# guokiddo1/speech_enhancement

Hardware: AMD Instinct MI355X
Metric: NoiseSup frames/sec (16 kHz, hop 80, 256-pt rfft, two-stage Wiener), batched (higher is better)
Workload: dtype f32; 1 GPU; BASELINE configs[1]: 1024-utterance batch per GPU, 256-pt rfft + two-stage Wiener NoiseSup (etsi_denoise semantics), SURVEY 8(d) synthetic 16 kHz corpus, 2-6 s utterances; utterances_per_gpu=1024, devices_visible=1

## Files before the change

### speech_enhancement_amd/csrc/ns6_beat_plan.h

```cpp
#ifndef SEA_NS6_BEAT_PLAN_H
#define SEA_NS6_BEAT_PLAN_H

#if defined(__HIPCC__) || defined(__CUDACC__)
#define SEA_NS6_HD __host__ __device__
#else
#define SEA_NS6_HD
#endif

namespace sea {
namespace ns6plan {

constexpr int kNoOnset = 0x7fffffff;
constexpr int kDepth = 9;

enum Role { FA = 0, FB = 1, B0 = 2, N1 = 3, G1 = 4, S = 5, kRoles = 6 };

constexpr unsigned kAlways = 0u, kFd = 1u, kLight = 2u, kDifg1 = 4u;
constexpr unsigned kRedeal = 8u;
constexpr unsigned kVariantPlain = kLight | kDifg1, kVariantDense = 0u, kVariantFd = kFd | kLight | kDifg1;
constexpr unsigned kVariantDenseRedeal = kRedeal;
constexpr unsigned kBin64 = 16u;
constexpr unsigned kVariantDenseBin64 = kRedeal | kBin64;
constexpr unsigned kIdctS = 32u;
constexpr unsigned kVariantDenseIdct = kRedeal | kBin64 | kIdctS;
constexpr int kDepthIdct = 12;

struct Flag {
    int d;
    int k;
    unsigned when;
};
constexpr int kMaxFlags = 5;
struct RolePlan {
    int n;
    Flag f[kMaxFlags];
    int ahead;
    int settle;
};

constexpr RolePlan kPlan[kRoles] = {
    {4, {{0, 3, kAlways}, {3, 5, kAlways}, {2, 1, kLight}, {3, 3, kRedeal}, {0, 0, 0}}, 1, 0},
    {2, {{1, 3, kAlways}, {4, 5, kAlways}, {0, 0, 0}, {0, 0, 0}, {0, 0, 0}}, 0, 0},
    {2, {{2, 3, kAlways}, {6, 5, kBin64}, {0, 0, 0}, {0, 0, 0}, {0, 0, 0}}, 0, 0},
    {3, {{5, 5, kAlways}, {7, 5, kAlways}, {2, 1, kRedeal}, {0, 0, 0}, {0, 0, 0}}, 0, 0},
    {1, {{8, 5, kAlways}, {0, 0, 0}, {0, 0, 0}, {0, 0, 0}, {0, 0, 0}}, 0, 0},
    {5, {{1, 1, kAlways}, {3, 3, kAlways}, {6, 5, kAlways}, {kDepth, 5, kAlways}, {kDepth, 5, kFd}}, 0, 1},
};

constexpr RolePlan kPlanIdct[kRoles] = {
    {3, {{0, 3, kAlways}, {4, 5, kAlways}, {4, 3, kAlways}, {0, 0, 0}, {0, 0, 0}}, 1, 0},
    {2, {{1, 3, kAlways}, {5, 5, kAlways}, {0, 0, 0}, {0, 0, 0}, {0, 0, 0}}, 0, 0},
    {2, {{2, 3, kAlways}, {7, 5, kAlways}, {0, 0, 0}, {0, 0, 0}, {0, 0, 0}}, 0, 0},
    {3, {{2, 1, kAlways}, {6, 5, kAlways}, {8, 5, kAlways}, {0, 0, 0}, {0, 0, 0}}, 0, 0},
    {2, {{9, 5, kAlways}, {11, 5, kAlways}, {0, 0, 0}, {0, 0, 0}, {0, 0, 0}}, 0, 0},
    {5, {{1, 1, kAlways}, {3, 3, kAlways}, {7, 5, kAlways}, {10, 5, kAlways}, {kDepthIdct, 5, kAlways}}, 0, 1},
};
SEA_NS6_HD constexpr const RolePlan &plan_of(unsigned variant, int role) { return (variant & kIdctS) ? kPlanIdct[role] : kPlan[role]; }
SEA_NS6_HD constexpr int depth_of(unsigned variant) { return (variant & kIdctS) ? kDepthIdct : kDepth; }

SEA_NS6_HD constexpr bool flag_applies(const Flag &f, unsigned variant) { return f.when == kAlways || (f.when & variant) != 0u; }

SEA_NS6_HD constexpr bool has_flag(unsigned variant, int role, int d, int k)
{
    const RolePlan &p = plan_of(variant, role);
    for (int j = 0; j < p.n; ++j)
        if (p.f[j].d == d && p.f[j].k == k && flag_applies(p.f[j], variant)) return true;
    return false;
}

SEA_NS6_HD constexpr int steady_lead(unsigned variant, int role)
{
    const RolePlan &p = plan_of(variant, role);
    int lead = 0;
    for (int j = 0; j < p.n; ++j) {
        const Flag &f = p.f[j];
        if (flag_applies(f, variant) && f.d + f.k - 1 > lead) lead = f.d + f.k - 1;
    }
    return lead + p.settle;
}
SEA_NS6_HD constexpr int steady_tail(unsigned variant, int role)
{
    const RolePlan &p = plan_of(variant, role);
    int tail = depth_of(variant);
    for (int j = 0; j < p.n; ++j) {
        const Flag &f = p.f[j];
        if (flag_applies(f, variant) && f.d < tail) tail = f.d;
    }
    return tail - p.ahead;
}

SEA_NS6_HD constexpr int steady_begin(unsigned variant, int role, int onset)
{
    return onset == kNoOnset ? kNoOnset : onset + steady_lead(variant, role);
}
SEA_NS6_HD constexpr int steady_end(unsigned variant, int role, int nfr)
{
    const int e = nfr + steady_tail(variant, role);
    return e > 0 ? e : 0;
}

}
}

#undef SEA_NS6_HD
#endif
```

### speech_enhancement_amd/csrc/ns_core.h

```cpp
#pragma once
#include "sea_device.h"
#include "sea_kernels.h"

namespace sea {

namespace {

constexpr int kRing = 320;
constexpr double kLn2 = 0.69314718055994530942;

struct __attribute__((aligned(16))) BackLds {
    float wbuf[68];
    float sbuf[68];
    float sq[80];
    float mel[28];
    float fir[20];
};

struct __attribute__((aligned(16))) NsLds {
    float ring[2][kRing];
    float work[256];
    float psd[68];
    BackLds back;
    float outb[80];
// ... 1359 lines not shown
    B.wbuf[lane] = WLo;
    if (lane == 0) B.wbuf[64] = WHi;
    wave_sync();
    float melOut = ns_mel_fb(B, C, lane);
    melOut = (float)((double)(alfaGF * melOut) + (1.0 - (double)alfaGF) * 1.0);
    float d0, d1;
    lastIn = ns_fir_dif_rl(fir_taps_rl(ns_idct_tap_rl_batch(melOut, C.irWin, lane, idctLds)), buf, lane, lastIn, d0, d1);
    if (lane < 40) *reinterpret_cast<float2 *>(dif + 2 * lane) = make_float2(d0, d1);
    wave_sync();
}

constexpr int kIdctRecFloats = 40;
__device__ __forceinline__ void ns_fir_from_idct_rec(const float *rec, float irWin, const float *buf, int lane, float &y0, float &y1)
{
    const int l = (lane <= 8) ? lane : 8;
    ns_fir_regs(fir_taps_rl(rec[28 + l] * irWin), buf, lane, y0, y1);
}
__device__ __forceinline__ void ns_fir_from_idct_taps(const float *taps, const float *buf, int lane, float &y0, float &y1)
{
    const FirTaps T = fir_taps_rl(taps[kIdsTapStride * lane]);
    constexpr int kFirst = 5;
    float x[18];
    int o = 72 + 2 * ((lane < 40) ? lane : 39);
#pragma unroll
    for (int m = 8; m < 18; m += 2) {
        const float2 v = *reinterpret_cast<const float2 *>(buf + o + m);
        x[m] = v.x;
        x[m + 1] = v.y;
    }
    __builtin_amdgcn_sched_barrier(0);
    y0 = 0.0f, y1 = 0.0f;
#pragma unroll
    for (int k = 0; k < kFirst; ++k) {
        const float c = T.t[8 - k];
        y0 += c * x[16 - k];
        y1 += c * x[17 - k];
    }
    asm("" : "+v"(o) : "v"(y0));
#pragma unroll
    for (int m = 0; m < 8; m += 2) {
        const float2 v = *reinterpret_cast<const float2 *>(buf + o + m);
        x[m] = v.x;
        x[m + 1] = v.y;
    }
    __builtin_amdgcn_sched_barrier(0);
#pragma unroll
    for (int k = kFirst; k < SEA_NTAP; ++k) {
        const float c = T.t[k < 8 ? 8 - k : k - 8];
        y0 += c * x[16 - k];
        y1 += c * x[17 - k];
    }
}

template <int ST, bool FD = false>
__device__ __forceinline__ void ns_stage(NsLds &L, NsRegs &s, const NsConst &C, int lane, NsFd *fd = nullptr,
                                         int *fdFlags = nullptr)
{
    ns_front(L.ring[ST], L.work, L.psd, C.fft, C.win, lane);
    ns_back<ST, false, FD, false, -1, true>(L.psd, L.ring[ST], L.back, s, C, (ST == 0) ? (L.ring[1] + 240) : L.outb, lane, 0.0f, nullptr,
                           nullptr, fd, fdFlags);
}

__device__ __forceinline__ bool dc_filter(const float *dif, float *out, float &yState, int lane)
{
    const float y0 = yState;
    float y = y0;
#pragma unroll 5
    for (int n = 0; n < SEA_HOP; n += 4) {
        const float4 d = *reinterpret_cast<const float4 *>(&dif[n]);
        float4 o;
        y = __fmaf_rn(0.9990234375f, y, d.x);
        o.x = y;
        y = __fmaf_rn(0.9990234375f, y, d.y);
        o.y = y;
        y = __fmaf_rn(0.9990234375f, y, d.z);
        o.z = y;
        y = __fmaf_rn(0.9990234375f, y, d.w);
        o.w = y;
        *reinterpret_cast<float4 *>(&out[n]) = o;
    }
    wave_sync();
    bool unsafe = false;
#pragma unroll
    for (int k = 0; k < 2; ++k) {
        const int n = lane + 64 * k;
        if (n < SEA_HOP) {
            const float ad = fabsf(dif[n]);
            const float ay = fabsf(n == 0 ? y0 : out[n - 1]);
            const bool ok = (ad == 0.0f) || (ay == 0.0f) ||
                            (ay >= ad * 0x1p-16f && ay <= ad * 0x1p26f && ad < 0x1p100f && ad > 0x1p-100f);
            unsafe |= !ok;
        }
    }
    const bool redo = __ballot(unsafe) != 0ull;
    if (redo) {
        wave_sync();
        y = y0;
        for (int n = 0; n < SEA_HOP; ++n) {
            y = (float)__fma_rn(0.9990234375, (double)y, (double)dif[n]);
            out[n] = y;
        }
    }
    yState = y;
    wave_sync();
    return redo;
}
// ... 295 lines not shown
```

### speech_enhancement_amd/csrc/ns_pipe6_kernel.hip

```cpp
#include "ns_core.h"
#include "ns6_beat_plan.h"

namespace sea {

namespace p6 {

#ifdef SEA_NS6_TIMING
__device__ unsigned long long g_ns6_timing[16];
struct RoleTimer6 {
    unsigned long long work = 0, wait = 0, t0 = 0, t1 = 0;
    __device__ __forceinline__ void begin() { t0 = clock64(); }
    __device__ __forceinline__ void mid() { t1 = clock64(); work += t1 - t0; }
    __device__ __forceinline__ void end() { wait += clock64() - t1; }
};
#define NS6_T_DECL RoleTimer6 rt_
#define NS6_T_BEGIN rt_.begin()
#define NS6_T_MID rt_.mid()
#define NS6_T_END rt_.end()
#define NS6_T_FLUSH(r, n) do { if (blockIdx.x == 0 && (threadIdx.x & 63) == 0) { g_ns6_timing[2 * (r)] = rt_.work; g_ns6_timing[2 * (r) + 1] = rt_.wait; g_ns6_timing[12] = (unsigned long long)(n); } } while (0)
#else
#define NS6_T_DECL
#define NS6_T_BEGIN
#define NS6_T_MID
#define NS6_T_END
#define NS6_T_FLUSH(r, n)
#endif

constexpr int kSlots = 8;
constexpr int kSlots1 = 16;
constexpr int kSlotLen = SEA_HOP;
constexpr int kCirc = kSlots * kSlotLen;
constexpr int kCirc1 = kSlots1 * kSlotLen;
constexpr int kMirror = 3 * kSlotLen;
constexpr int kWaves = 6;
constexpr int kDepth = ns6plan::kDepth;
constexpr int kSChunks = 10;
constexpr int kPrioStep = 16;
constexpr int kPrioLevels = 32;
constexpr int kDefaultPerm = 0014352;
constexpr int kRedealPerm = 0140325;

constexpr int kNoOnset = ns6plan::kNoOnset;
constexpr long long kMaxFrames = 0x7fffffffLL - 16;
__device__ __forceinline__ void onset_poll(int &onset, const int *word)
{
    if (onset == kNoOnset)
        onset = __builtin_amdgcn_readfirstlane(__hip_atomic_load(word, __ATOMIC_RELAXED, __HIP_MEMORY_SCOPE_WORKGROUP));
}
__device__ __forceinline__ int tick_of(int f, int onset) { return (int)((unsigned)f - (unsigned)onset + 1u); }
__device__ __forceinline__ bool tick_ge(int f, int k, int onset, int nfr) { return f < nfr && f - (k - 1) >= onset; }

template <bool B>
struct BoolC {
    static constexpr bool value = B;
};
template <unsigned VARIANT, int ROLE, int D, int K, bool STEADY>
__device__ __forceinline__ bool beat_flag(int i, int onset, int nfr)
{
    static_assert(ns6plan::has_flag(VARIANT, ROLE, D, K), "a flag the beat plan of ns6_beat_plan.h does not know");
    return STEADY || tick_ge(i - D, K, onset, nfr);
}
struct NoEnter {
    __device__ __forceinline__ int operator()(int h) const { return h; }
};
template <bool STEADY_LOOP, unsigned VARIANT, int ROLE, bool PAIRED = false, class Beat, class Enter = NoEnter>
__device__ __forceinline__ void run_beats(int niter, int nfr, const int &onset, Beat &&beat, Enter &&enter = Enter{})
{
    int i = 0;
    while (i < niter) {
        if (STEADY_LOOP && i >= ns6plan::steady_begin(VARIANT, ROLE, onset)) {
            const int e0 = ns6plan::steady_end(VARIANT, ROLE, nfr), e = e0 < niter ? e0 : niter;
            if constexpr (PAIRED) {
                if ((i & 1) == 0) {
                    int h = enter(i >> 1);
                    for (const int he = e >> 1; h < he; ++h) {
                        beat(BoolC<true>{}, 2 * h);
                        beat(BoolC<true>{}, 2 * h + 1);
                    }
                    i = 2 * h;
                }
            } else
                for (; i < e; ++i) beat(BoolC<true>{}, i);
        }
        if (i < niter) {
            beat(BoolC<false>{}, i);
            ++i;
        }
    }
}

constexpr int kP1Ring = 8;
constexpr int kRnRing = 4;
constexpr int kW1Ring = 4;
struct __attribute__((aligned(16))) RecPsd {
    float psd[68];
};
struct __attribute__((aligned(16))) RecDen {
    float den[68];
};
struct __attribute__((aligned(16))) RecN {
    float P[68], noise[68];
};
struct __attribute__((aligned(16))) RecOut {
    float out[80];
};

struct __attribute__((aligned(16))) RecTap {
    float rec[kIdctRecFloats];
};

struct __attribute__((aligned(16))) Pipe6Lds {
    float circ0[kCirc + kMirror];
    float circ1[kCirc1 + kMirror];
    float work[2][512];
    BackLds back[2];
    float ssq[80], sdif[80], sout[80], szero[4];
    float frameEn[kSlots], denSum[kSlots];
    int onset;
    float frameEnLog[kSlots];
    int fdFlags[kSlots];
    float idctT[SEA_NMEL * 16];
    RecPsd p0[2], p1[kP1Ring];
    RecDen rd[2];
    RecN rn[kRnRing];
    RecOut ro[2];
    float nzSum[2], alfa[2];
    RecTap tap[2];
    float w1hi[kW1Ring];
};
constexpr bool lds_slots_differ(size_t a, size_t b) { return (a % 256) != (b % 256); }
#define NS6_OFF(m) offsetof(Pipe6Lds, m)
static_assert(lds_slots_differ(NS6_OFF(ssq), NS6_OFF(rd[0].den)) && lds_slots_differ(NS6_OFF(ssq), NS6_OFF(rd[1].den)), "ssq | den");
static_assert(lds_slots_differ(NS6_OFF(sdif), NS6_OFF(rn[0].noise)) && lds_slots_differ(NS6_OFF(sdif), NS6_OFF(rn[1].noise)) &&
              lds_slots_differ(NS6_OFF(sdif), NS6_OFF(rn[2].noise)) && lds_slots_differ(NS6_OFF(sdif), NS6_OFF(rn[3].noise)), "sdif | noise");
static_assert(lds_slots_differ(NS6_OFF(ro[0].out), NS6_OFF(rn[1].noise)) && lds_slots_differ(NS6_OFF(ro[0].out), NS6_OFF(rn[3].noise)) &&
              lds_slots_differ(NS6_OFF(ro[1].out), NS6_OFF(rn[0].noise)) && lds_slots_differ(NS6_OFF(ro[1].out), NS6_OFF(rn[2].noise)), "ro | noise");
static_assert(lds_slots_differ(NS6_OFF(ssq[68]), NS6_OFF(szero)) && lds_slots_differ(NS6_OFF(ssq[72]), NS6_OFF(szero)) &&
              lds_slots_differ(NS6_OFF(ssq[76]), NS6_OFF(szero)), "ssq tail | szero");
static_assert(lds_slots_differ(NS6_OFF(sdif[68]), NS6_OFF(szero)) && lds_slots_differ(NS6_OFF(sdif[72]), NS6_OFF(szero)) &&
              lds_slots_differ(NS6_OFF(sdif[76]), NS6_OFF(szero)), "sdif tail | szero");
static_assert(lds_slots_differ(NS6_OFF(ro[0].out[68]), NS6_OFF(szero)) && lds_slots_differ(NS6_OFF(ro[0].out[72]), NS6_OFF(szero)) &&
              lds_slots_differ(NS6_OFF(ro[0].out[76]), NS6_OFF(szero)) && lds_slots_differ(NS6_OFF(ro[1].out[68]), NS6_OFF(szero)) &&
              lds_slots_differ(NS6_OFF(ro[1].out[72]), NS6_OFF(szero)) && lds_slots_differ(NS6_OFF(ro[1].out[76]), NS6_OFF(szero)), "ro tail | szero");
#undef NS6_OFF
static_assert(sizeof(Pipe6Lds) == 24960 && 4 * sizeof(Pipe6Lds) <= 160 * 1024 && sizeof(Pipe6Lds) < 40 * 1024,
              "the figure in the comment at kP1Ring; four workgroups fit a CU");

struct __attribute__((aligned(16))) Pipe6Idct {
    float tap[2][2][kIdsTapFloats];
    float pad0[4];
    float zeros[kIdsZeros];
    float pad[4];
    float prod[2][2][kIdctProdFloats];
};
constexpr int kIdctBasisAt = 3;
struct __attribute__((aligned(16))) Pipe6LdsIdct {
    Pipe6Lds base;
    Pipe6Idct x;
};
constexpr size_t lds_slot(size_t off) { return (off / 16) % 16; }
constexpr bool lds_group_ok(size_t ssq, size_t den, size_t recA, size_t recB, int r0, int r1)
{
    size_t sl[11] = {lds_slot(ssq), lds_slot(den)};
    int n = 2;
    for (int r = 0; r < 9; ++r) sl[n++] = lds_slot(((r >= r0 && r < r1) ? recA : recB) + r * kIdctStride * sizeof(float));
    for (int i = 0; i < n; ++i)
        for (int j = i + 1; j < n; ++j)
            if (sl[i] == sl[j]) return false;
    return true;
}
#define NS6_OFF(m) offsetof(Pipe6LdsIdct, m)
static_assert(NS6_OFF(base) == 0 && NS6_OFF(x.prod) % 256 == NS6_OFF(x.prod[0][1]) % 256 && NS6_OFF(x.prod) % 256 == NS6_OFF(x.prod[1][0]) % 256 &&
                  NS6_OFF(x.prod) % 256 == NS6_OFF(x.prod[1][1]) % 256 && NS6_OFF(x.prod) % 16 == 0 && (kIdctRow * sizeof(float)) % 16 == 0 &&
                  (NS6_OFF(base.idctT) + kIdctBasisAt * sizeof(float)) % 16 == 0 && kIdctBasisAt + kIdctBasisFloats <= SEA_NMEL * 16 &&
                  NS6_OFF(x.tap[0][1]) % 16 == 0 && NS6_OFF(x.tap[1][1]) + kIdsTapReach * sizeof(float) <= sizeof(Pipe6LdsIdct),
              "the four product records share their slots");
static_assert(lds_group_ok(NS6_OFF(base.ssq), NS6_OFF(base.rd[0].den), NS6_OFF(x.prod[0][0]), NS6_OFF(x.prod[1][1]), 0, 3) &&
                  lds_group_ok(NS6_OFF(base.ssq), NS6_OFF(base.rd[0].den), NS6_OFF(x.prod[0][0]), NS6_OFF(x.prod[1][1]), 3, 9) &&
                  lds_group_ok(NS6_OFF(base.ssq), NS6_OFF(base.rd[1].den), NS6_OFF(x.prod[0][1]), NS6_OFF(x.prod[1][0]), 0, 3) &&
                  lds_group_ok(NS6_OFF(base.ssq), NS6_OFF(base.rd[1].den), NS6_OFF(x.prod[0][1]), NS6_OFF(x.prod[1][0]), 3, 9) &&
                  (kIdctStride * sizeof(float)) % 16 == 0, "n < 28: ssq, den | the rows, in both groups and both parities");
static_assert(NS6_OFF(x.zeros) % 16 == 0 && lds_slots_differ(NS6_OFF(x.zeros) + 256 - kIdctRow * sizeof(float), NS6_OFF(base.ssq)) &&
                  lds_slots_differ(NS6_OFF(x.zeros) + 256 - kIdctRow * sizeof(float), NS6_OFF(base.rd[0].den)) &&
                  lds_slots_differ(NS6_OFF(x.zeros) + 256 - kIdctRow * sizeof(float), NS6_OFF(base.rd[1].den)), "28 <= n: the rows' zeros | ssq, den");
static_assert(lds_slots_differ(NS6_OFF(x.zeros) + 512 - 68 * sizeof(float), NS6_OFF(base.ssq)) &&
                  lds_slots_differ(NS6_OFF(x.zeros) + 512 - 68 * sizeof(float), NS6_OFF(base.sdif)) &&
                  lds_slots_differ(NS6_OFF(x.zeros) + 512 - 68 * sizeof(float), NS6_OFF(x.zeros) + 256 - kIdctRow * sizeof(float)),
              "68 <= n: the den and noise lanes' zeros | ssq, sdif, the rows' zeros");
#undef NS6_OFF
static_assert(4 * sizeof(Pipe6LdsIdct) <= 160 * 1024 && 5 * sizeof(Pipe6LdsIdct) <= 160 * 1024, "four workgroups fit a CU; five, for the compiler's occupancy of 7");

template <int SLOTS>
__device__ __forceinline__ int window_base(int tick) { return ((tick - 3) & (SLOTS - 1)) * kSlotLen; }

template <int SLOTS>
__device__ __forceinline__ void slot_store(float *circ, int tick, int lane, float a, float b)
{
    const int slot = tick & (SLOTS - 1);
    float *p = circ + slot * kSlotLen + 2 * lane;
    *reinterpret_cast<float2 *>(p) = make_float2(a, b);
    if (slot < 3) *reinterpret_cast<float2 *>(p + SLOTS * kSlotLen) = make_float2(a, b);
}

__device__ __forceinline__ void block_sync()
{
    __builtin_amdgcn_fence(__ATOMIC_RELEASE, "workgroup", "local");
    __builtin_amdgcn_s_barrier();
    __builtin_amdgcn_fence(__ATOMIC_ACQUIRE, "workgroup", "local");
}

__device__ __forceinline__ void load_back_const(NsConst &C, const sea_ns_tables *t, int lane)
{
    C.melStart = t->melStart[lane];
    C.melLen = t->melLen[lane];
#pragma unroll
    for (int i = 0; i < SEA_MEL_TAPS; ++i) C.melW[i] = t->melW[i][lane];
    C.irWin = t->irWin[lane];
    C.eps = t->eps;
}

template <bool FD, bool LIGHT , bool DIFG1 ,
          bool STEADY_LOOP ,
          bool REDEAL = false ,
          bool BIN64 = false ,
          bool IDCTS = false ,
          bool PAIRED = false >
__device__ __forceinline__ void ns_pipe6_body(const NsBatchArgs &a, Pipe6Lds &L, Pipe6Idct *X = nullptr)
{
    static_assert(!REDEAL || (!LIGHT && !DIFG1), "the re-deal is a variant of the dense body");
    static_assert(!BIN64 || (REDEAL && !FD), "the guest of B0's second component is a variant of the re-dealt dense body");
    static_assert(!IDCTS || BIN64, "the IDCT sums in the helper wave are a variant of that body in turn");
    static_assert(!PAIRED || STEADY_LOOP, "the paired beats are the steady copies'");
    constexpr unsigned V = (FD ? ns6plan::kFd : 0u) | (LIGHT ? ns6plan::kLight : 0u) | (DIFG1 ? ns6plan::kDifg1 : 0u) | (REDEAL ? ns6plan::kRedeal : 0u) |
                           (BIN64 ? ns6plan::kBin64 : 0u) | (IDCTS ? ns6plan::kIdctS : 0u);
    static_assert(!BIN64 || V == (IDCTS ? ns6plan::kVariantDenseIdct : ns6plan::kVariantDenseBin64),
                  "the variants tests/test_ns6_idct_plan_cpu.py and tests/test_ns6_bin64_plan_cpu.py sweep");
    constexpr int kS1 = IDCTS ? 1 : 0;
    constexpr int DEPTH = ns6plan::depth_of(V);
    static_assert(DEPTH == (IDCTS ? 12 : kDepth), "the depth the ring depths at kP1Ring are derived for");
    constexpr bool LOG_N1 = REDEAL, FIR_FA = REDEAL;
    const int lane = threadIdx.x & 63;
    const int role = ((a.perm6 ? a.perm6 : (REDEAL ? kRedealPerm : kDefaultPerm)) >> (3 * __builtin_amdgcn_readfirstlane(threadIdx.x >> 6))) & 7;
    const int u = a.order ? a.order[blockIdx.x] : (int)blockIdx.x;
    const long long off = a.offsets[u];
    const long long nfr64 = a.lengths[u] / SEA_HOP;
    const int nfr = __builtin_amdgcn_readfirstlane((int)(nfr64 < kMaxFrames ? nfr64 : kMaxFrames));
    const int niter = nfr + DEPTH;
    const bool lrpt = a.prio_row > 0 && a.order;
    const long long longestFr = lrpt ? a.lengths[a.order[0]] / SEA_HOP : 0;
    const float lrptScale = (float)kPrioLevels / (float)(longestFr > 0 ? longestFr : 1);
    const int lrptBias = lrpt ? (int)blockIdx.x / a.prio_row : 0;
    auto prio_by_remaining = [&](int i) {
        if ((FD ? lrpt : true) && (i & (kPrioStep - 1)) == 0) {
            if constexpr (!FD) {
                asm volatile("");
                if (!lrpt) return;
            }
            const int L = __builtin_amdgcn_readfirstlane((int)((float)(nfr - i) * lrptScale)) + lrptBias;
            const int pr = (L + (int)(((unsigned)i / kPrioStep) & (kPrioLevels / 4 - 1))) / (kPrioLevels / 4);
            if (pr >= 3) __builtin_amdgcn_s_setprio(3);
            else if (pr == 2) __builtin_amdgcn_s_setprio(2);
            else if (pr == 1) __builtin_amdgcn_s_setprio(1);
            else __builtin_amdgcn_s_setprio(0);
        }
    };

    {
        static_assert(offsetof(Pipe6Lds, circ0) == 0 && offsetof(Pipe6Lds, circ1) == sizeof(float) * (kCirc + kMirror), "circ0 | circ1 lead the record");
        float *z = reinterpret_cast<float *>(&L);
        for (int i = threadIdx.x; i < kCirc + kCirc1 + 2 * kMirror; i += 64 * kWaves) z[i] = 0.0f;
    }
    if constexpr (!IDCTS)
        for (int i = threadIdx.x; i < SEA_NMEL * 16; i += 64 * kWaves) L.idctT[i] = a.tables->idct[i >> 4][i & 15];
    float *const basisQ = L.idctT + kIdctBasisAt;
    if (threadIdx.x < 4) L.szero[threadIdx.x] = 0.0f;
    if (threadIdx.x < kSlots) {
        L.frameEn[threadIdx.x] = 0.0f;
        L.frameEnLog[threadIdx.x] = 0.0f;
        L.denSum[threadIdx.x] = 0.0f;
    }
    if (threadIdx.x < 2) {
        const int k = threadIdx.x;
        L.rd[k].den[65] = L.rd[k].den[66] = L.rd[k].den[67] = 0.0f;
        L.nzSum[k] = L.alfa[k] = 0.0f;
    }
    if (threadIdx.x < kRnRing) {
        const int k = threadIdx.x;
        L.rn[k].noise[65] = L.rn[k].noise[66] = L.rn[k].noise[67] = 0.0f;
    }
    if (threadIdx.x == 0) L.onset = kNoOnset;
    if constexpr (IDCTS) {
        for (int i = threadIdx.x; i < kIdctBasisFloats; i += 64 * kWaves) {
            const int t = i / kIdctRow, f = i % kIdctRow;
            basisQ[i] = (t < 9 && f < SEA_NMEL) ? a.tables->idct[f][t] : 0.0f;
        }
        if (threadIdx.x < kIdsZeros) X->zeros[threadIdx.x] = 0.0f;
        if (threadIdx.x < 6) L.back[threadIdx.x / 3].mel[SEA_NMEL + threadIdx.x % 3] = 0.0f;
    }
    block_sync();
    NS6_T_DECL;

    if (role == 0) {
        Fft2Regs fft;
        load_fft2_regs<false>(fft, &a.tables->fft, lane, nullptr);
        float win8[8];
#pragma unroll
        for (int k = 0; k < 8; ++k) win8[k] = a.tables->win8[k][lane];
        const float irWin = (FIR_FA && !IDCTS) ? a.tables->irWin[lane] : 0.0f;
        const uint32_t *in32 = reinterpret_cast<const uint32_t *>(a.in + off);
        uint32_t nextw = (lane < 40 && nfr > 0) ? in32[lane] : 0u;
        int onsetG = kNoOnset;
        int onsetS = kNoOnset;
        typedef const __attribute__((address_space(1))) uint32_t *FramePtr;
        unsigned long long nextFr = 0;
        auto beat = [&](auto steady, int i) __attribute__((always_inline)) {
            constexpr bool STEADY = decltype(steady)::value;
            int &onset = *(STEADY && PAIRED ? &onsetS : &onsetG);
            constexpr bool NEXT_S = STEADY && PAIRED;
            NS6_T_BEGIN;
            prio_by_remaining(i);
            if constexpr (LIGHT) {
                if (beat_flag<V, ns6plan::FA, 2, 1, STEADY>(i, onset, nfr)) {
                    const int e = (tick_of(i - 2, onset) + 2) & (kSlots - 1);
                    const float en = vad_frame_energy(L.frameEn[e]);
                    if (lane == 0) L.frameEnLog[e] = en;
                }
            }
            int tick = 0;
            bool actA = false;
            if (STEADY || i < nfr) {
                const uint32_t w = nextw;
                if constexpr (!NEXT_S)
                    if ((STEADY || i + 1 < nfr) && lane < 40) nextw = (in32 + (long long)(i + 1) * 40)[lane];
                if (!STEADY && onset == kNoOnset && __ballot(w != 0u) != 0ull) {
                    onset = i;
                    if (lane == 0) __hip_atomic_store(&L.onset, i, __ATOMIC_RELAXED, __HIP_MEMORY_SCOPE_WORKGROUP);
                }
                if (STEADY || i >= onset) {
                    tick = tick_of(i, onset);
                    const float x0 = (float)(short)(w & 0xFFFFu), x1 = (float)(short)(w >> 16);
                    if (lane < 40) {
                        if constexpr (NEXT_S) nextw = reinterpret_cast<FramePtr>(nextFr)[lane];
                        slot_store<kSlots>(L.circ0, tick, lane, x0, x1);
                    }
                    if constexpr (NEXT_S) {
                        nextFr += SEA_HOP * 2u;
                        asm("" : "+s"(nextFr));
                    }
                    static_assert(ns6plan::has_flag(V, ns6plan::FA, 0, 3), "frame i exists here: its flag is the tick alone");
                    actA = STEADY || tick >= 3;
                }
            }
            const int t1 = tick_of(i - 3 - kS1, onset);
            const bool actB = beat_flag<V, ns6plan::FA, 3 + kS1, 5, STEADY>(i, onset, nfr);
            if constexpr (FIR_FA) {
                if (beat_flag<V, ns6plan::FA, 3 + kS1, 3, STEADY>(i, onset, nfr)) {
                    float y0, y1;
                    if constexpr (IDCTS)
                        ns_fir_from_idct_taps(X->tap[0][(i - 4) & 1], L.circ0 + window_base<kSlots>(t1), lane, y0, y1);
                    else
                        ns_fir_from_idct_rec(L.tap[(i - 3) & 1].rec, irWin, L.circ0 + window_base<kSlots>(t1), lane, y0, y1);
                    if (lane < 40) slot_store<kSlots1>(L.circ1, t1, lane, y0, y1);
                    wave_sync();
                }
            }
            if (actA || actB) {
                wave_sync();
                float e[8];
                ns_window8(L.circ0 + window_base<kSlots>(tick), actA, L.circ1 + window_base<kSlots1>(t1), actB, win8, lane, e);
                if constexpr (STEADY && PAIRED && !FD) {
#pragma unroll
                    for (int q = 0; q < 4; ++q) asm volatile("" : "+v"(fft.head8[q]));
                }
                rfft256_dual_lo<false>(e, L.work[i & 1], fft);
            }
            NS6_T_MID;
            block_sync();
            NS6_T_END;
        };
        run_beats<STEADY_LOOP, V, ns6plan::FA, PAIRED>(niter, nfr, onsetG, beat, [&](int h) {
            onsetS = __builtin_amdgcn_readfirstlane(onsetG);
            const int hs = __builtin_amdgcn_readfirstlane(h);
            unsigned long long fr = reinterpret_cast<unsigned long long>(in32 + (unsigned long long)(unsigned)(2 * hs + 1) * 40u);
            asm("" : "+s"(fr));
            nextFr = fr;
            return hs;
        });
        NS6_T_FLUSH(role, niter);
        if (FD && a.onset_out && lane == 0) a.onset_out[u] = onsetG == kNoOnset ? nfr : onsetG;
    } else if (role == 1) {
        Fft2Regs fft;
        load_fft2_regs<false>(fft, &a.tables->fft, lane, nullptr);
        int onset = kNoOnset;
        auto beat = [&](auto steady, int i) __attribute__((always_inline)) {
            constexpr bool STEADY = decltype(steady)::value;
            NS6_T_BEGIN;
            prio_by_remaining(i);
            if (!STEADY) onset_poll(onset, &L.onset);
            const int g = i - 1;
            if (STEADY || g >= 0) {
                const int f0 = g, f1 = g - 3 - kS1;
                const bool actA = beat_flag<V, ns6plan::FB, 1, 3, STEADY>(i, onset, nfr);
                const bool actB = beat_flag<V, ns6plan::FB, 4 + kS1, 5, STEADY>(i, onset, nfr);
                float *work = L.work[g & 1];
                if (actA || actB) {
                    float o[8];
                    rfft256_dual_hi_keep_last<false>(work, fft, o);
                    psd_from_last_level(o, fft, L.p0[f0 & 1].psd, actA, L.p1[f1 & (kP1Ring - 1)].psd, actB, lane);
// ... 39 lines not shown
                if constexpr (IDCTS) {
                    ns_back<0, true, FD, true, SEA_NMEL, false, true, true, true>(r.psd, nullptr, L.back[0], s, C, X->prod[0][f & 1], lane, frameEn, o.den,
                                                                                  basisQ, &fd, &bits, nullptr, nullptr, nullptr, &x);
                } else if constexpr (BIN64) {
                    ns_back<0, true, FD, true, SEA_NMEL, false, true, true>(r.psd, nullptr, L.back[0], s, C, L.tap[f & 1].rec, lane, frameEn, o.den,
                                                                            L.idctT, &fd, &bits, nullptr, nullptr, nullptr, &x);
                } else if constexpr (FIR_FA) {
                    ns_back<0, true, FD, true, SEA_NMEL, false, true>(r.psd, nullptr, L.back[0], s, C, L.tap[f & 1].rec, lane, frameEn, o.den, L.idctT,
                                                         &fd, &bits);
                    if (FD && lane == 0) L.fdFlags[t & (kSlots - 1)] = bits;
                } else {
                    float y01[2] = {0.0f, 0.0f};
                    ns_back<0, true, FD, true, -1, false, true>(r.psd, L.circ0 + window_base<kSlots>(t), L.back[0], s, C, nullptr, lane, frameEn, o.den,
                                               L.idctT, &fd, &bits, nullptr, y01);
                    if (FD && lane == 0) L.fdFlags[t & (kSlots - 1)] = bits;
                    if (lane < 40) slot_store<kSlots1>(L.circ1, t, lane, y01[0], y01[1]);
                }
            }
            if constexpr (BIN64) {
                if (x.live) {
                    if (!x.done) {
                        const float W = gain_bin<false>(sqrtf(x.P1[64]), sqrtf(x.psd1[64]), x.noise1[64], x.den);
                        x.W = W;
                    }
                    if (lane == 1) L.w1hi[g & (kW1Ring - 1)] = x.W;
                }
            }
            NS6_T_MID;
            block_sync();
            NS6_T_END;
        };
        run_beats<STEADY_LOOP, V, ns6plan::B0, PAIRED>(niter, nfr, onset, beat);
        NS6_T_FLUSH(role, niter);
    } else if (role == 3) {
        const float eps = a.tables->eps;
        NsRegs s;
        regs_init(s, eps);
        int onset = kNoOnset;
        auto beat = [&](auto steady, int i) __attribute__((always_inline)) {
            constexpr bool STEADY = decltype(steady)::value;
            NS6_T_BEGIN;
            prio_by_remaining(i);
            if (!STEADY) onset_poll(onset, &L.onset);
            const int f = i - 5 - kS1, fg = i - 7 - kS1;
            if constexpr (LOG_N1) {
                if (beat_flag<V, ns6plan::N1, 2, 1, STEADY>(i, onset, nfr)) {
                    const int e = (tick_of(i - 2, onset) + 2) & (kSlots - 1);
                    const float en = vad_frame_energy(L.frameEn[e]);
                    if (lane == 0) L.frameEnLog[e] = en;
                }
            }
            if (beat_flag<V, ns6plan::N1, 7 + kS1, 5, STEADY>(i, onset, nfr)) {
                const int t = tick_of(fg, onset);
                s.denEn0 = L.denSum[(t - 2) & (kSlots - 1)];
                s.denEn1 = L.denSum[(t - 1) & (kSlots - 1)];
                s.denEn2 = L.denSum[t & (kSlots - 1)];
                const int nbNow = s.nbFrame[1];
                s.nbFrame[1] = t - 4;
                gain_fact_update(s, L.nzSum[fg & 1]);
                s.nbFrame[1] = nbNow;
                if (lane == 0) L.alfa[fg & 1] = s.alfaGF;
            }
            if (beat_flag<V, ns6plan::N1, 5 + kS1, 5, STEADY>(i, onset, nfr)) {
                const RecPsd &r = L.p1[f & (kP1Ring - 1)];
                RecN &o = L.rn[f & (kRnRing - 1)];
                ns_noise1<BIN64>(r.psd, o.P, o.noise, s, eps, lane);
            }
            NS6_T_MID;
            block_sync();
            NS6_T_END;
        };
        run_beats<STEADY_LOOP, V, ns6plan::N1, PAIRED>(niter, nfr, onset, beat);
        NS6_T_FLUSH(role, niter);
    } else if (role == 4) {
        NsConst C;
        load_back_const(C, a.tables, lane);
        NsRegs s;
        regs_init(s, C.eps);
        float lastIn = 0.0f;
        int onset = kNoOnset;
        auto beat = [&](auto steady, int i) __attribute__((always_inline)) {
            constexpr bool STEADY = decltype(steady)::value;
            NS6_T_BEGIN;
            prio_by_remaining(i);
            if (!STEADY) onset_poll(onset, &L.onset);
            const int f = i - 8 - kS1;
            if constexpr (IDCTS) {
                const int ff = i - 11;
                if (beat_flag<V, ns6plan::G1, 11, 5, STEADY>(i, onset, nfr))
                    ns_fir_from_taps(X->tap[1][ff & 1], L.back[1].fir, L.circ1 + window_base<kSlots1>(tick_of(ff, onset)), L.ro[ff & 1].out, lane);
            }
            if (beat_flag<V, ns6plan::G1, 8 + kS1, 5, STEADY>(i, onset, nfr)) {
                const float *psd = L.p1[f & (kP1Ring - 1)].psd;
                const RecN &r = L.rn[f & (kRnRing - 1)];
                RecOut &o = L.ro[f & 1];
                const int t = tick_of(f, onset);
                const float alfa = L.alfa[f & 1];
                const float *w64 = BIN64 ? &L.w1hi[f & (kW1Ring - 1)] : nullptr;
                if constexpr (IDCTS)
                    ns_gain1_products(psd, r.P, r.noise, alfa, L.back[1], s, C, X->prod[1][f & 1], lane, basisQ, w64);
                else if (DIFG1)
                    ns_gain1_dif(psd, r.P, r.noise, alfa, L.circ1 + window_base<kSlots1>(t), L.back[1], s, C, o.out, lane, L.idctT, lastIn);
                else
                    ns_gain1<BIN64>(psd, r.P, r.noise, alfa, L.circ1 + window_base<kSlots1>(t), L.back[1], s, C, o.out, lane, L.idctT, w64);
            }
            NS6_T_MID;
            block_sync();
            NS6_T_END;
        };
        run_beats<STEADY_LOOP, V, ns6plan::G1, PAIRED>(niter, nfr, onset, beat);
        NS6_T_FLUSH(role, niter);
    } else {
        uint32_t *out32 = reinterpret_cast<uint32_t *>(a.out + off);
        float *outf = a.out_f32 ? a.out_f32 + off : nullptr;
        float dcX = 0.0f, dcY = 0.0f;
        int firstOut = -1;
        int onset = kNoOnset;
        HelperIdct ids = {};
        if constexpr (IDCTS) {
            static_assert(!IDCTS || !DIFG1, "the DC lanes read sdif");
            char *const lds = reinterpret_cast<char *>(&L);
            auto at = [&](const void *q) { return (int)(reinterpret_cast<const char *>(q) - lds); };
            const int g = lane >> 4, t = (lane - 1) & 15;
            const bool row = t <= 8 && g <= 1;
            constexpr int kProd = sizeof(X->prod[0][0]), kTap = sizeof(X->tap[0][0]), kRowB = kIdctStride * sizeof(float), kTapB = kIdsTapStride * sizeof(float);
            ids.lds = lds;
            ids.rowZeros = at(X->zeros) - kIdctRow * (int)sizeof(float);
            if (row) {
                ids.src0 = (g == 0 ? at(X->prod[0][0]) : at(X->prod[1][1])) + kRowB * t;
                ids.srcP = g == 0 ? kProd : -kProd;
                ids.end = ids.rowZeros;
                ids.tap0 = (g == 0 ? at(X->tap[0][0]) : at(X->tap[1][1])) + kTapB * t;
                ids.tapP = g == 0 ? kTap : -kTap;
            } else {
                ids.src0 = g == 0 ? at(L.ssq) : (g == 1 ? at(L.rd[0].den) : (g == 2 ? at(L.sdif) : at(L.rn[0].noise)));
                ids.srcP = g == 1 ? (int)sizeof(RecDen) : 0;
                ids.srcQ = g == 3 ? (int)sizeof(RecN) : 0;
                ids.end = (g == 1 || g == 3) ? at(X->zeros) - 68 * (int)sizeof(float) : ids.src0;
            }
            ids.hann = a.tables->irWin[t];
            ids.m = g == 2 ? 0.9990234375f : 1.0f;
            ids.acc0 = (g == 0 && !row) ? 64.0f : 0.0f;
        }
        auto beat = [&](auto steady, int i) __attribute__((always_inline)) {
            constexpr bool STEADY = decltype(steady)::value;
            NS6_T_BEGIN;
            prio_by_remaining(i);
            if (!STEADY) onset_poll(onset, &L.onset);
            const int fp = i - 1, fd = i - 3, fn = i - 6 - kS1, fo = i - DEPTH;
            const bool doVad = beat_flag<V, ns6plan::S, 1, 1, STEADY>(i, onset, nfr), doDen = beat_flag<V, ns6plan::S, 3, 3, STEADY>(i, onset, nfr),
                       doNz = beat_flag<V, ns6plan::S, 6 + kS1, 5, STEADY>(i, onset, nfr), produced = beat_flag<V, ns6plan::S, DEPTH, 5, STEADY>(i, onset, nfr);
            bool doIdct1 = false;
            if constexpr (IDCTS) doIdct1 = beat_flag<V, ns6plan::S, 10, 5, STEADY>(i, onset, nfr);
            const int tp = tick_of(fp, onset), td = tick_of(fd, onset);
            const float *denSrc = L.rd[(STEADY || (fd >= 0 && fd < nfr)) ? (fd & 1) : 0].den;
            const float *nzSrc = L.rn[fn & (kRnRing - 1)].noise;
            const bool haveOut = STEADY || (fo >= 0 && fo < nfr);
            float2 vOut = make_float2(0.0f, 0.0f);
            const int l2 = (lane < 40) ? lane : 39;
            float2 sqIn = *reinterpret_cast<const float2 *>(L.circ0 + (tp & (kSlots - 1)) * kSlotLen + 2 * l2);
            const float *difS = DIFG1 ? L.ro[fo & 1].out : L.sdif;
            if constexpr (DIFG1) {
                asm volatile("" : "+v"(sqIn.x), "+v"(sqIn.y));
            } else {
                const float *y2 = L.ro[fo & 1].out;
                float2 yIn = *reinterpret_cast<const float2 *>(y2 + 2 * l2);
                float below = y2[(l2 > 0) ? 2 * l2 - 1 : 0], last = y2[79];
                asm volatile("" : "+v"(sqIn.x), "+v"(sqIn.y), "+v"(yIn.x), "+v"(yIn.y), "+v"(below), "+v"(last));
                if (produced) {
                    const float xm1 = (lane == 0) ? dcX : below;
                    *reinterpret_cast<float2 *>(L.sdif + 2 * l2) = make_float2(yIn.x - xm1, yIn.y - yIn.x);
                    dcX = last;
                }
            }
            if (doVad) *reinterpret_cast<float2 *>(L.ssq + 2 * l2) = make_float2(sqIn.x * sqIn.x, sqIn.y * sqIn.y);
            if (doVad || doDen || doNz || doIdct1 || produced) {
                wave_sync();
                float vadSum, denTotal, nzTotal, y = dcY;
                if constexpr (IDCTS) {
                    static_assert(((10 - 3) & 1) == 1, "S's two product records of a beat have opposite frame parities");
                    ids.p = fd & 1;
                    ids.q = fn & (kRnRing - 1);
                    helper_chains<kSChunks, false, true, true>(L.ssq, denSrc, difS, L.sout, L.szero, vadSum, denTotal, y, lane, nullptr, nullptr,
                                                               nullptr, nzSrc, &nzTotal, &ids);
                } else
                    helper_chains<kSChunks, false, true>(L.ssq, denSrc, difS, L.sout, L.szero, vadSum, denTotal, y, lane, nullptr, nullptr,
                                                         nullptr, nzSrc, &nzTotal);
                if (doVad) {
                    const float en = (LIGHT || LOG_N1) ? vadSum : vad_frame_energy(vadSum);
                    if (lane == 0) L.frameEn[(tp + 2) & (kSlots - 1)] = en;
                }
                if (doDen && lane == 0) L.denSum[td & (kSlots - 1)] = denTotal;
                if (doNz && lane == 0) L.nzSum[fn & 1] = nzTotal;
                if (produced) {
                    vOut = dc_verify_take(difS, L.sout, dcY, y, lane);
                    dcY = y;
                    if (!STEADY && firstOut < 0) firstOut = fo;
                }
            }
            if (haveOut) {
                if (lane < 40) {
                    uint32_t packed = 0u;
                    if (produced) {
                        packed = (uint32_t)cast_i16(vOut.x) | ((uint32_t)cast_i16(vOut.y) << 16);
                        if (outf) *reinterpret_cast<float2 *>(outf + (long long)fo * SEA_HOP + 2 * lane) = vOut;
                    }
                    (out32 + (long long)fo * 40)[lane] = packed;
                }
                if constexpr (FD) {
                    if (beat_flag<V, ns6plan::S, DEPTH, 5, STEADY>(i, onset, nfr) && lane == 0 && a.flags_out)
                        a.flags_out[off / 8 + 10 * (long long)fo] = (unsigned char)L.fdFlags[tick_of(fo, onset) & (kSlots - 1)];
                }
                wave_sync();
            }
            NS6_T_MID;
            block_sync();
            NS6_T_END;
        };
        run_beats<STEADY_LOOP, V, ns6plan::S, PAIRED>(niter, nfr, onset, beat);
        NS6_T_FLUSH(role, niter);
        if (a.first_out && lane == 0) a.first_out[u] = firstOut;
    }
}

}

__global__ __launch_bounds__(384, 6) void ns_denoise_pipe6_kernel(NsBatchArgs a)
{
    __shared__ p6::Pipe6Lds L;
    p6::ns_pipe6_body<false, true, true, true, false, false, false, true>(a, L);
}
#ifdef SEA_NS6_TIMING
__device__ unsigned g_ns6_wg[16384 * 4];
#endif
__global__ __launch_bounds__(384, 7) void ns_denoise_pipe6_dense_kernel(NsBatchArgs a)
{
    __shared__ p6::Pipe6LdsIdct L;
#ifdef SEA_NS6_TIMING
    if (threadIdx.x == 0 && blockIdx.x < 16384) {
        g_ns6_wg[4 * blockIdx.x] = (unsigned)wall_clock64();
        g_ns6_wg[4 * blockIdx.x + 2] = __builtin_amdgcn_s_getreg((31 << 11) | (0 << 6) | 4);
        g_ns6_wg[4 * blockIdx.x + 3] = __builtin_amdgcn_s_getreg((31 << 11) | (0 << 6) | 20);
    }
#endif
    p6::ns_pipe6_body<false, false, false, true, true, true, true, true>(a, L.base, &L.x);
#ifdef SEA_NS6_TIMING
    if (threadIdx.x == 0 && blockIdx.x < 16384) g_ns6_wg[4 * blockIdx.x + 1] = (unsigned)wall_clock64();
#endif
}
__global__ __launch_bounds__(384, 2) void ns_denoise_pipe6_fd_kernel(NsBatchArgs a)
{
    __shared__ p6::Pipe6Lds L;
    p6::ns_pipe6_body<true, true, true, true, false, false, false, true>(a, L);
}

}

#ifdef SEA_NS6_TIMING
extern "C" int sea_debug_ns6_timing(unsigned long long *out16)
{
    return (int)hipMemcpyFromSymbol(out16, HIP_SYMBOL(sea::p6::g_ns6_timing), 16 * sizeof(unsigned long long));
}
extern "C" int sea_debug_ns6_wg(unsigned *out, int n_wg)
{
    return (int)hipMemcpyFromSymbol(out, HIP_SYMBOL(sea::g_ns6_wg), (size_t)n_wg * 4 * sizeof(unsigned));
}
#endif
```

Baseline: 610.7 million frames/s.

## Merge both stages' FIR passes into one paired wave pass in dense pipeline

Adds a FIRP variant of the dense six-wave pipeline. Both Wiener stages' FIR filtering now runs in the G1 wave in a single call, with half the lanes doing each stage and three outputs per lane. The FA wave's own FIR pass is removed, and the beat plan is re-staged to depth 13 with a new role permutation and a 16-entry denSum ring. The goal is to rebalance work across the waves so FA is lighter. In exchange the pipeline gets deeper, with more fill and drain beats per utterance.

Measured after the change: 641.7 million frames/s, median of 6. 5.1% higher.

```diff
diff --git a/speech_enhancement_amd/csrc/ns6_beat_plan.h b/speech_enhancement_amd/csrc/ns6_beat_plan.h
--- a/speech_enhancement_amd/csrc/ns6_beat_plan.h
+++ b/speech_enhancement_amd/csrc/ns6_beat_plan.h
@@ -24,6 +24,9 @@
 constexpr unsigned kIdctS = 32u;
 constexpr unsigned kVariantDenseIdct = kRedeal | kBin64 | kIdctS;
 constexpr int kDepthIdct = 12;
+constexpr unsigned kFirPair = 64u;
+constexpr unsigned kVariantDenseFirPair = kRedeal | kBin64 | kIdctS | kFirPair;
+constexpr int kDepthFirPair = 13;
 
 struct Flag {
     int d;
@@ -55,8 +58,19 @@
     {2, {{9, 5, kAlways}, {11, 5, kAlways}, {0, 0, 0}, {0, 0, 0}, {0, 0, 0}}, 0, 0},
     {5, {{1, 1, kAlways}, {3, 3, kAlways}, {7, 5, kAlways}, {10, 5, kAlways}, {kDepthIdct, 5, kAlways}}, 0, 1},
 };
-SEA_NS6_HD constexpr const RolePlan &plan_of(unsigned variant, int role) { return (variant & kIdctS) ? kPlanIdct[role] : kPlan[role]; }
-SEA_NS6_HD constexpr int depth_of(unsigned variant) { return (variant & kIdctS) ? kDepthIdct : kDepth; }
+constexpr RolePlan kPlanFirPair[kRoles] = {
+    {2, {{0, 3, kAlways}, {5, 5, kAlways}, {0, 0, 0}, {0, 0, 0}, {0, 0, 0}}, 1, 0},
+    {2, {{1, 3, kAlways}, {6, 5, kAlways}, {0, 0, 0}, {0, 0, 0}, {0, 0, 0}}, 0, 0},
+    {2, {{2, 3, kAlways}, {8, 5, kAlways}, {0, 0, 0}, {0, 0, 0}, {0, 0, 0}}, 0, 0},
+    {3, {{2, 1, kAlways}, {7, 5, kAlways}, {9, 5, kAlways}, {0, 0, 0}, {0, 0, 0}}, 0, 0},
+    {3, {{4, 3, kAlways}, {10, 5, kAlways}, {12, 5, kAlways}, {0, 0, 0}, {0, 0, 0}}, 0, 0},
+    {5, {{1, 1, kAlways}, {3, 3, kAlways}, {8, 5, kAlways}, {11, 5, kAlways}, {kDepthFirPair, 5, kAlways}}, 0, 1},
+};
+SEA_NS6_HD constexpr const RolePlan &plan_of(unsigned variant, int role)
+{
+    return (variant & kFirPair) ? kPlanFirPair[role] : ((variant & kIdctS) ? kPlanIdct[role] : kPlan[role]);
+}
+SEA_NS6_HD constexpr int depth_of(unsigned variant) { return (variant & kFirPair) ? kDepthFirPair : ((variant & kIdctS) ? kDepthIdct : kDepth); }
 
 SEA_NS6_HD constexpr bool flag_applies(const Flag &f, unsigned variant) { return f.when == kAlways || (f.when & variant) != 0u; }
 
diff --git a/speech_enhancement_amd/csrc/ns_core.h b/speech_enhancement_amd/csrc/ns_core.h
--- a/speech_enhancement_amd/csrc/ns_core.h
+++ b/speech_enhancement_amd/csrc/ns_core.h
@@ -1435,6 +1435,48 @@
     }
 }
 
+struct FirPair3 {
+    char *lds;
+    int x;
+    int tap;
+    int dst;
+};
+__device__ __forceinline__ void ns_fir_pair3(const FirPair3 &F, int win0, int win1 , int tapPar ,
+                                             int dst0, int dst1 ,
+                                             int mirror, bool live0, bool live1, int lane)
+{
+    const bool hi = lane >= 32;
+    const bool third = (lane & 31) < 26;
+    const float *taps = reinterpret_cast<const float *>(F.lds + (F.tap + tapPar));
+    const float *src = reinterpret_cast<const float *>(F.lds + (F.x + (hi ? win1 : win0)));
+    float *dst = reinterpret_cast<float *>(F.lds + (F.dst + (hi ? dst1 : dst0)));
+    float t[9], x[19];
+#pragma unroll
+    for (int k = 0; k < 9; ++k) t[k] = taps[kIdsTapStride * k];
+#pragma unroll
+    for (int m = 0; m < 19; ++m) x[m] = src[m];
+    float y0 = 0.0f, y1 = 0.0f, y2 = 0.0f;
+#pragma unroll
+    for (int k = 0; k < SEA_NTAP; ++k) {
+        const float c = t[k < 8 ? 8 - k : k - 8];
+        y0 += c * x[16 - k];
+        y1 += c * x[17 - k];
+        y2 += c * x[18 - k];
+    }
+    const bool live = hi ? live1 : live0;
+    if (live) {
+        dst[0] = y0;
+        dst[1] = y1;
+        if (third) dst[2] = y2;
+    }
+    if (mirror > 0 && live0 && !hi) {
+        float *m = reinterpret_cast<float *>(reinterpret_cast<char *>(dst) + mirror);
+        m[0] = y0;
+        m[1] = y1;
+        if (third) m[2] = y2;
+    }
+}
+
 template <int ST, bool FD = false>
 __device__ __forceinline__ void ns_stage(NsLds &L, NsRegs &s, const NsConst &C, int lane, NsFd *fd = nullptr,
                                          int *fdFlags = nullptr)
diff --git a/speech_enhancement_amd/csrc/ns_pipe6_kernel.hip b/speech_enhancement_amd/csrc/ns_pipe6_kernel.hip
--- a/speech_enhancement_amd/csrc/ns_pipe6_kernel.hip
+++ b/speech_enhancement_amd/csrc/ns_pipe6_kernel.hip
@@ -38,7 +38,7 @@
 constexpr int kPrioStep = 16;
 constexpr int kPrioLevels = 32;
 constexpr int kDefaultPerm = 0014352;
-constexpr int kRedealPerm = 0140325;
+constexpr int kRedealPerm = 0104325;
 
 constexpr int kNoOnset = ns6plan::kNoOnset;
 constexpr long long kMaxFrames = 0x7fffffffLL - 16;
@@ -92,6 +92,7 @@
 constexpr int kP1Ring = 8;
 constexpr int kRnRing = 4;
 constexpr int kW1Ring = 4;
+constexpr int kDenRing16 = 16;
 struct __attribute__((aligned(16))) RecPsd {
     float psd[68];
 };
@@ -152,6 +153,7 @@
     float zeros[kIdsZeros];
     float pad[4];
     float prod[2][2][kIdctProdFloats];
+    float denSum16[kDenRing16];
 };
 constexpr int kIdctBasisAt = 3;
 struct __attribute__((aligned(16))) Pipe6LdsIdct {
@@ -180,6 +182,11 @@
                   lds_group_ok(NS6_OFF(base.ssq), NS6_OFF(base.rd[1].den), NS6_OFF(x.prod[0][1]), NS6_OFF(x.prod[1][0]), 0, 3) &&
                   lds_group_ok(NS6_OFF(base.ssq), NS6_OFF(base.rd[1].den), NS6_OFF(x.prod[0][1]), NS6_OFF(x.prod[1][0]), 3, 9) &&
                   (kIdctStride * sizeof(float)) % 16 == 0, "n < 28: ssq, den | the rows, in both groups and both parities");
+static_assert(lds_group_ok(NS6_OFF(base.ssq), NS6_OFF(base.rd[0].den), NS6_OFF(x.prod[0][0]), NS6_OFF(x.prod[1][0]), 0, 3) &&
+                  lds_group_ok(NS6_OFF(base.ssq), NS6_OFF(base.rd[0].den), NS6_OFF(x.prod[0][0]), NS6_OFF(x.prod[1][0]), 3, 9) &&
+                  lds_group_ok(NS6_OFF(base.ssq), NS6_OFF(base.rd[1].den), NS6_OFF(x.prod[0][1]), NS6_OFF(x.prod[1][1]), 0, 3) &&
+                  lds_group_ok(NS6_OFF(base.ssq), NS6_OFF(base.rd[1].den), NS6_OFF(x.prod[0][1]), NS6_OFF(x.prod[1][1]), 3, 9),
+              "the same with both stages' records of one parity");
 static_assert(NS6_OFF(x.zeros) % 16 == 0 && lds_slots_differ(NS6_OFF(x.zeros) + 256 - kIdctRow * sizeof(float), NS6_OFF(base.ssq)) &&
                   lds_slots_differ(NS6_OFF(x.zeros) + 256 - kIdctRow * sizeof(float), NS6_OFF(base.rd[0].den)) &&
                   lds_slots_differ(NS6_OFF(x.zeros) + 256 - kIdctRow * sizeof(float), NS6_OFF(base.rd[1].den)), "28 <= n: the rows' zeros | ssq, den");
@@ -224,20 +231,24 @@
           bool REDEAL = false ,
           bool BIN64 = false ,
           bool IDCTS = false ,
-          bool PAIRED = false >
+          bool PAIRED = false ,
+          bool FIRP = false >
 __device__ __forceinline__ void ns_pipe6_body(const NsBatchArgs &a, Pipe6Lds &L, Pipe6Idct *X = nullptr)
 {
     static_assert(!REDEAL || (!LIGHT && !DIFG1), "the re-deal is a variant of the dense body");
     static_assert(!BIN64 || (REDEAL && !FD), "the guest of B0's second component is a variant of the re-dealt dense body");
     static_assert(!IDCTS || BIN64, "the IDCT sums in the helper wave are a variant of that body in turn");
     static_assert(!PAIRED || STEADY_LOOP, "the paired beats are the steady copies'");
+    static_assert(!FIRP || IDCTS, "the merged filter pass takes both stages' taps from the helper wave");
     constexpr unsigned V = (FD ? ns6plan::kFd : 0u) | (LIGHT ? ns6plan::kLight : 0u) | (DIFG1 ? ns6plan::kDifg1 : 0u) | (REDEAL ? ns6plan::kRedeal : 0u) |
-                           (BIN64 ? ns6plan::kBin64 : 0u) | (IDCTS ? ns6plan::kIdctS : 0u);
-    static_assert(!BIN64 || V == (IDCTS ? ns6plan::kVariantDenseIdct : ns6plan::kVariantDenseBin64),
-                  "the variants tests/test_ns6_idct_plan_cpu.py and tests/test_ns6_bin64_plan_cpu.py sweep");
-    constexpr int kS1 = IDCTS ? 1 : 0;
+                           (BIN64 ? ns6plan::kBin64 : 0u) | (IDCTS ? ns6plan::kIdctS : 0u) | (FIRP ? ns6plan::kFirPair : 0u);
+    static_assert(!BIN64 || V == (FIRP ? ns6plan::kVariantDenseFirPair : (IDCTS ? ns6plan::kVariantDenseIdct : ns6plan::kVariantDenseBin64)),
+                  "the variants tests/test_ns6_fir_plan_cpu.py, tests/test_ns6_idct_plan_cpu.py and tests/test_ns6_bin64_plan_cpu.py sweep");
+    constexpr int kS1 = FIRP ? 2 : (IDCTS ? 1 : 0);
     constexpr int DEPTH = ns6plan::depth_of(V);
-    static_assert(DEPTH == (IDCTS ? 12 : kDepth), "the depth the ring depths at kP1Ring are derived for");
+    static_assert(DEPTH == (FIRP ? 13 : (IDCTS ? 12 : kDepth)) && DEPTH == 9 + 2 * (IDCTS ? 1 : 0) + kS1, "the depth the ring depths at kP1Ring are derived for");
+    constexpr int kDenRing = FIRP ? kDenRing16 : kSlots;
+    float *const denRing = FIRP ? X->denSum16 : L.denSum;
     constexpr bool LOG_N1 = REDEAL, FIR_FA = REDEAL;
     const int lane = threadIdx.x & 63;
     const int role = ((a.perm6 ? a.perm6 : (REDEAL ? kRedealPerm : kDefaultPerm)) >> (3 * __builtin_amdgcn_readfirstlane(threadIdx.x >> 6))) & 7;
@@ -295,6 +306,7 @@
             basisQ[i] = (t < 9 && f < SEA_NMEL) ? a.tables->idct[f][t] : 0.0f;
         }
         if (threadIdx.x < kIdsZeros) X->zeros[threadIdx.x] = 0.0f;
+        if (FIRP && threadIdx.x < kDenRing16) X->denSum16[threadIdx.x] = 0.0f;
         if (threadIdx.x < 6) L.back[threadIdx.x / 3].mel[SEA_NMEL + threadIdx.x % 3] = 0.0f;
     }
     block_sync();
@@ -353,7 +365,7 @@
             }
             const int t1 = tick_of(i - 3 - kS1, onset);
             const bool actB = beat_flag<V, ns6plan::FA, 3 + kS1, 5, STEADY>(i, onset, nfr);
-            if constexpr (FIR_FA) {
+            if constexpr (FIR_FA && !FIRP) {
                 if (beat_flag<V, ns6plan::FA, 3 + kS1, 3, STEADY>(i, onset, nfr)) {
                     float y0, y1;
                     if constexpr (IDCTS)
@@ -499,9 +511,9 @@
             }
             if (beat_flag<V, ns6plan::N1, 7 + kS1, 5, STEADY>(i, onset, nfr)) {
                 const int t = tick_of(fg, onset);
-                s.denEn0 = L.denSum[(t - 2) & (kSlots - 1)];
-                s.denEn1 = L.denSum[(t - 1) & (kSlots - 1)];
-                s.denEn2 = L.denSum[t & (kSlots - 1)];
+                s.denEn0 = denRing[(t - 2) & (kDenRing - 1)];
+                s.denEn1 = denRing[(t - 1) & (kDenRing - 1)];
+                s.denEn2 = denRing[t & (kDenRing - 1)];
                 const int nbNow = s.nbFrame[1];
                 s.nbFrame[1] = t - 4;
                 gain_fact_update(s, L.nzSum[fg & 1]);
@@ -526,13 +538,32 @@
         regs_init(s, C.eps);
         float lastIn = 0.0f;
         int onset = kNoOnset;
+        FirPair3 fp = {};
+        if constexpr (FIRP) {
+            char *const lds = reinterpret_cast<char *>(&L);
+            auto at = [&](const void *q) { return (int)(reinterpret_cast<const char *>(q) - lds); };
+            const int j = (lane & 31) < 27 ? (lane & 31) : 26;
+            fp.lds = lds;
+            fp.x = (lane < 32 ? at(L.circ0) : at(L.circ1)) + (72 + 3 * j) * (int)sizeof(float);
+            fp.tap = lane < 32 ? at(X->tap[0][0]) : at(X->tap[1][0]);
+            fp.dst = (lane < 32 ? at(L.circ1) : at(L.ro[0].out)) + 3 * j * (int)sizeof(float);
+        }
         auto beat = [&](auto steady, int i) __attribute__((always_inline)) {
             constexpr bool STEADY = decltype(steady)::value;
             NS6_T_BEGIN;
             prio_by_remaining(i);
             if (!STEADY) onset_poll(onset, &L.onset);
             const int f = i - 8 - kS1;
-            if constexpr (IDCTS) {
+            if constexpr (FIRP) {
+                const int f0 = i - 4, f1 = i - 12;
+                const bool live0 = beat_flag<V, ns6plan::G1, 4, 3, STEADY>(i, onset, nfr), live1 = beat_flag<V, ns6plan::G1, 12, 5, STEADY>(i, onset, nfr);
+                if (live0 || live1) {
+                    const int t0 = tick_of(f0, onset), slot = t0 & (kSlots1 - 1);
+                    constexpr int kF = sizeof(float);
+                    ns_fir_pair3(fp, window_base<kSlots>(t0) * kF, window_base<kSlots1>(tick_of(f1, onset)) * kF, (f0 & 1) * (int)sizeof(X->tap[0][0]),
+                                 slot * kSlotLen * kF, (f1 & 1) * (int)sizeof(RecOut), slot < 3 ? kCirc1 * kF : 0, live0, live1, lane);
+                }
+            } else if constexpr (IDCTS) {
                 const int ff = i - 11;
                 if (beat_flag<V, ns6plan::G1, 11, 5, STEADY>(i, onset, nfr))
                     ns_fir_from_taps(X->tap[1][ff & 1], L.back[1].fir, L.circ1 + window_base<kSlots1>(tick_of(ff, onset)), L.ro[ff & 1].out, lane);
@@ -574,11 +605,11 @@
             ids.lds = lds;
             ids.rowZeros = at(X->zeros) - kIdctRow * (int)sizeof(float);
             if (row) {
-                ids.src0 = (g == 0 ? at(X->prod[0][0]) : at(X->prod[1][1])) + kRowB * t;
-                ids.srcP = g == 0 ? kProd : -kProd;
+                ids.src0 = (g == 0 ? at(X->prod[0][0]) : at(X->prod[1][FIRP ? 0 : 1])) + kRowB * t;
+                ids.srcP = (g == 0 || FIRP) ? kProd : -kProd;
                 ids.end = ids.rowZeros;
-                ids.tap0 = (g == 0 ? at(X->tap[0][0]) : at(X->tap[1][1])) + kTapB * t;
-                ids.tapP = g == 0 ? kTap : -kTap;
+                ids.tap0 = (g == 0 ? at(X->tap[0][0]) : at(X->tap[1][FIRP ? 0 : 1])) + kTapB * t;
+                ids.tapP = (g == 0 || FIRP) ? kTap : -kTap;
             } else {
                 ids.src0 = g == 0 ? at(L.ssq) : (g == 1 ? at(L.rd[0].den) : (g == 2 ? at(L.sdif) : at(L.rn[0].noise)));
                 ids.srcP = g == 1 ? (int)sizeof(RecDen) : 0;
@@ -598,7 +629,7 @@
             const bool doVad = beat_flag<V, ns6plan::S, 1, 1, STEADY>(i, onset, nfr), doDen = beat_flag<V, ns6plan::S, 3, 3, STEADY>(i, onset, nfr),
                        doNz = beat_flag<V, ns6plan::S, 6 + kS1, 5, STEADY>(i, onset, nfr), produced = beat_flag<V, ns6plan::S, DEPTH, 5, STEADY>(i, onset, nfr);
             bool doIdct1 = false;
-            if constexpr (IDCTS) doIdct1 = beat_flag<V, ns6plan::S, 10, 5, STEADY>(i, onset, nfr);
+            if constexpr (IDCTS) doIdct1 = beat_flag<V, ns6plan::S, FIRP ? 11 : 10, 5, STEADY>(i, onset, nfr);
             const int tp = tick_of(fp, onset), td = tick_of(fd, onset);
             const float *denSrc = L.rd[(STEADY || (fd >= 0 && fd < nfr)) ? (fd & 1) : 0].den;
             const float *nzSrc = L.rn[fn & (kRnRing - 1)].noise;
@@ -625,7 +656,7 @@
                 wave_sync();
                 float vadSum, denTotal, nzTotal, y = dcY;
                 if constexpr (IDCTS) {
-                    static_assert(((10 - 3) & 1) == 1, "S's two product records of a beat have opposite frame parities");
+                    static_assert((((FIRP ? 11 : 10) - 3) & 1) == (FIRP ? 0 : 1), "S's two product records of a beat have opposite frame parities; FIRP: the same");
                     ids.p = fd & 1;
                     ids.q = fn & (kRnRing - 1);
                     helper_chains<kSChunks, false, true, true>(L.ssq, denSrc, difS, L.sout, L.szero, vadSum, denTotal, y, lane, nullptr, nullptr,
@@ -637,7 +668,7 @@
                     const float en = (LIGHT || LOG_N1) ? vadSum : vad_frame_energy(vadSum);
                     if (lane == 0) L.frameEn[(tp + 2) & (kSlots - 1)] = en;
                 }
-                if (doDen && lane == 0) L.denSum[td & (kSlots - 1)] = denTotal;
+                if (doDen && lane == 0) denRing[td & (kDenRing - 1)] = denTotal;
                 if (doNz && lane == 0) L.nzSum[fn & 1] = nzTotal;
                 if (produced) {
                     vOut = dc_verify_take(difS, L.sout, dcY, y, lane);
@@ -690,7 +721,7 @@
         g_ns6_wg[4 * blockIdx.x + 3] = __builtin_amdgcn_s_getreg((31 << 11) | (0 << 6) | 20);
     }
 #endif
-    p6::ns_pipe6_body<false, false, false, true, true, true, true, true>(a, L.base, &L.x);
+    p6::ns_pipe6_body<false, false, false, true, true, true, true, true, true>(a, L.base, &L.x);
 #ifdef SEA_NS6_TIMING
     if (threadIdx.x == 0 && blockIdx.x < 16384) g_ns6_wg[4 * blockIdx.x + 1] = (unsigned)wall_clock64();
 #endif
```
